# cvigilv/SimSpread.jl

Hardware: AMD Instinct MI355X
Metric: predicted edges/sec + achieved HBM GB/s, W*R SpMM (higher is better)
Workload: dtype f32

## Files before the change

### simspread.jl_amd/csrc/api.hip

```cpp
#include <algorithm>
#include <cmath>
#include <cstdlib>
#include <mutex>
#include <new>
#include <shared_mutex>
#include <type_traits>

#include "graph.hpp"

namespace ss {

std::string& last_error() {
  static thread_local std::string msg;
  return msg;
}

int fail(int code, const char* fmt, ...) {
  char buf[1024];
  va_list ap;
  va_start(ap, fmt);
  vsnprintf(buf, sizeof(buf), fmt, ap);
  va_end(ap);
  last_error() = buf;
  return code;
// ... 175 lines not shown
  T* dst = W;
  int64_t sld = ld, dld = ldw;
  if (mem == SS_MEM_HOST) {
    SS_TRY(din.alloc((size_t)rows * cols));
    SS_TRY(dout.alloc((size_t)rows * cols));
    SS_HIP(hipMemcpy2DAsync(din.p, rows * sizeof(T), G, ld * sizeof(T), rows * sizeof(T), cols, hipMemcpyHostToDevice, st));
    src = din.p; dst = dout.p; sld = rows; dld = rows;
  }
  SS_TRY(launch_row_degree<T>(src, rows, cols, sld, deg.p));
  SS_TRY(launch_spread_dense<T>(src, rows, cols, sld, deg.p, dst, dld));
  if (mem == SS_MEM_HOST)
    SS_HIP(hipMemcpy2DAsync(W, ldw * sizeof(T), dout.p, rows * sizeof(T), rows * sizeof(T), cols, hipMemcpyDeviceToHost, st));
  SS_HIP(hipStreamSynchronize(st));
  return SS_OK;
}

struct HandleHead {
  int dtype;
  std::mutex mu;
};
static uint64_t next_graph_id() {
  static std::atomic<uint64_t> n{0};
  return ++n;
}
template <class T>
struct GraphBox : HandleHead {
  uint64_t id = next_graph_id();
  Graph<T> g;
};
template <class T>
struct QueriesBox : HandleHead {
  uint64_t graph_id = 0;
  DevCsr<T> Xq;
};
template <class T>
struct SpMatBox : HandleHead {
  SpMat<T> m;
};

template <class T>
static int graph_check(const void* h, Graph<T>** out) {
  if (!h) return fail(SS_EINVAL, "graph handle is NULL");
  GraphBox<T>* b = const_cast<GraphBox<T>*>(reinterpret_cast<const GraphBox<T>*>(h));
  if (b->dtype != (int)sizeof(T)) return fail(SS_EINVAL, "graph handle was created with the other precision");
  *out = &b->g;
  return SS_OK;
}

template <class T>
static int queries_check(const void* qh, const void* h, const DevCsr<T>** out) {
  const QueriesBox<T>* q = reinterpret_cast<const QueriesBox<T>*>(qh);
  if (q->dtype != (int)sizeof(T)) return fail(SS_EINVAL, "query set was created with the other precision");
  if (q->graph_id != reinterpret_cast<const GraphBox<T>*>(h)->id)
    return fail(SS_EINVAL, "query set was created for another graph");
  *out = &q->Xq;
  return SS_OK;
}

template <class T>
static int graph_create_csr_impl(int64_t nq, int64_t ns, int64_t nf, int64_t nt, const int64_t* xq_ptr,
                                 const int32_t* xq_idx, const T* xq_val, const int64_t* xs_ptr, const int32_t* xs_idx,
                                 const T* xs_val, const int64_t* ys_ptr, const int32_t* ys_idx, const T* ys_val,
                                 int index_base, int mem, ss_graph** out) {
  SS_TRY(require_init());
  SS_TRY(check_mem(mem));
  if (!out) return fail(SS_EINVAL, "out handle pointer is NULL");
  *out = nullptr;
  if (nq < 0 || ns < 0 || nf < 0 || nt < 0) return fail(SS_EINVAL, "negative node count");
  GraphBox<T>* box = new (std::nothrow) GraphBox<T>();
  if (!box) return fail(SS_ENOMEM, "host allocation failed");
  box->dtype = (int)sizeof(T);
  Graph<T>& g = box->g;
  g.nq = nq; g.ns = ns; g.nf = nf; g.nt = nt;
  int rc = csr_from_user<T>(nq, nf, xq_ptr, xq_idx, xq_val, index_base, mem, g.Xq);
  if (rc == SS_OK) rc = csr_from_user<T>(ns, nf, xs_ptr, xs_idx, xs_val, index_base, mem, g.Xs);
  if (rc == SS_OK) rc = csr_from_user<T>(ns, nt, ys_ptr, ys_idx, ys_val, index_base, mem, g.Ys);
  if (rc == SS_OK) rc = graph_finalize<T>(g);
  if (rc != SS_OK) { delete box; return rc; }
  *out = reinterpret_cast<ss_graph*>(box);
  return SS_OK;
}

template <class T>
static int graph_create_dense_impl(int64_t nq, int64_t ns, int64_t nf, int64_t nt, const T* Sq, int64_t ldq,
                                   const T* Ss, int64_t lds, const T* Y, int64_t ldy, int apply_cutoff, T alpha,
                                   int weighted, int mem, ss_graph** out) {
  SS_TRY(require_init());
  SS_TRY(check_mem(mem));
// ... 812 lines not shown
    StageTimer t2(ST_SPMM);
    SS_TRY(launch_spmm_sell<T>(W, R, ldr, nb, out, d.ld, kt_clean, rows));
    timing_count(ST_NSPMM, 1);
    return SS_OK;
  }
  const size_t nsorted = (size_t)rb * (size_t)W.vrows;
  const size_t need_s = nsorted + (rows ? (size_t)rb * (size_t)ncols : 0);
  if (ws.n < need_s) SS_TRY(ws.alloc(need_s));
  {
    StageTimer t2(ST_SPMM);
    SS_TRY(launch_spmm_sell<T>(W, R, ldr, nb, ws.p, W.vrows, nullptr));
    timing_count(ST_NSPMM, 1);
  }
  StageTimer t3(ST_EPILOGUE);
  T* packed = ws.p + nsorted;
  SS_TRY(launch_unpermute<T>(ws.p, W.vrows, nb, ncols, W.vfirst.p, W.inv.p, kt_clean, rows ? packed : out,
                             rows ? ncols : d.ld));
  if (d.host_rows) {
    for (int64_t q = 0; q < nb; ++q)
      SS_HIP(hipMemcpyAsync(d.dst + (int64_t)d.host_rows[d.o + q] * d.ld, packed + q * ncols, ncols * sizeof(T),
                            hipMemcpyDeviceToDevice, ctx().stream));
  } else if (rows) {
    SS_TRY(launch_scatter_rows<T>(packed, ncols, nb, ncols, rows, d.dst, d.ld));
  }
  return SS_OK;
}

template <class T>
static int stage2_rows(Graph<T>& g, int64_t rb, int64_t nb, const int* kt_clean, const ScoreDest<T>& d) {
  return sell_rows<T>(g.W, g.Tws.p, g.ns, g.nt, g.Sws, rb, nb, kt_clean, d);
}

template <class T>
static int predict_rows_device(Graph<T>& g, const DevCsr<T>& Xq, int kind, int64_t row_begin, int64_t row_end, int clean,
                               T* dev_out, int64_t ldo) {
  const int64_t nrows = row_end - row_begin;
  const int64_t nj = g.ns;
  SS_TRY(graph_sell(g));
  SS_TRY(graph_chunked(g, kind == SS_ROWS_SOURCE));
  const int64_t rb = transfer_batch_rows(nrows, nj, sizeof(T));
  const size_t need = (size_t)rb * (size_t)(nj > 0 ? nj : 1);
  if (g.Tws.n < need) SS_TRY(g.Tws.alloc(need));
  DevBuf<T>& Tbuf = g.Tws;
  for (int64_t r0 = 0; r0 < nrows; r0 += rb) {
    const int64_t nb = (nrows - r0 < rb) ? (nrows - r0) : rb;
    {
      StageTimer t1(ST_TRANSFER);
      if (g.dense.on) {
        const bool loo = (kind == 2);
        const bool srcrows = (kind == SS_ROWS_SOURCE);
        SS_TRY(dense_transfer<T>(g, loo, loo ? g.dense.inv_kf_m1.p : g.inv_kf.p, g.inv_ks.p, g.ks.p, row_begin + r0, nb,
                                 Tbuf.p, nj, srcrows, nullptr));
        if (srcrows) {
          const DevCsr<T>* L[2] = {&g.Ys, nullptr};
          const DevChunked<T>* M[2] = {&g.YsTc, nullptr};
          const T* inv1[2] = {g.inv_kt.p, nullptr};
          SS_TRY(launch_transfer<T>(1, L, inv1, M, g.inv_ks.p, row_begin + r0, nb, nj, Tbuf.p, nj, nullptr, true));
        }
      } else if (kind == 2) {
        SS_TRY(launch_transfer_loo<T>(g.Xs, g.XsTc, g.kf.p, g.ks.p, row_begin + r0, nb, Tbuf.p, nj));
      } else if (kind == SS_ROWS_QUERY) {
        const bool want_block = env_int("SS_TRANSFER_V", 0) >= 2 && transfer_block_fits<T>(g.XsT.rows, g.XsTc.SC);
        if (want_block) {
          if (g.XsTb.SC == 0) {
            const int al = env_int("SS_TRANSFER_ALIGN", 32) == 1 ? 1 : 32;
            SS_TRY(chunked_build<T>(g.XsT, g.XsTc.SC, al, g.XsTb));
          }
          if (g.Cq.n < (size_t)(Xq.nnz > 0 ? Xq.nnz : 1)) SS_TRY(g.Cq.alloc((size_t)(Xq.nnz > 0 ? Xq.nnz : 1)));
          const bool fixed = !env_off("SS_TRANSFER_FIX");
          SS_TRY(launch_transfer_block<T>(Xq, g.inv_kf.p, g.XsTb, g.inv_ks.p, row_begin + r0, nb, nj, Tbuf.p, nj, g.Cq.p,
                                          g.XsTb.vmax, fixed));
        } else {
          const DevCsr<T>* L[2] = {&Xq, nullptr};
          const DevChunked<T>* M[2] = {&g.XsTc, nullptr};
          const T* inv1[2] = {g.inv_kf.p, nullptr};
          SS_TRY(launch_transfer<T>(1, L, inv1, M, g.inv_ks.p, row_begin + r0, nb, nj, Tbuf.p, nj));
        }
      } else {
        const DevCsr<T>* L[2] = {&g.Xs, &g.Ys};
        const DevChunked<T>* M[2] = {&g.XsTc, &g.YsTc};
        const T* inv1[2] = {g.inv_kf.p, g.inv_kt.p};
        SS_TRY(launch_transfer<T>(2, L, inv1, M, g.inv_ks.p, row_begin + r0, nb, nj, Tbuf.p, nj));
      }
      timing_count(ST_NTRANSFER, 1);
    }
    SS_TRY(stage2_rows<T>(g, rb, nb, clean ? g.kt.p : nullptr, ScoreDest<T>{dev_out, ldo, r0, nullptr, nullptr}));
  }
  if (kind == 2 && clean) {
    StageTimer t3(ST_EPILOGUE);
    SS_TRY(launch_loo_clean_fix<T>(g.YsT, g.kt.p, row_begin, nrows, dev_out, ldo));
  }
  return SS_OK;
}

template <class T>
static int loo_graph_check(const Graph<T>& g) {
  if (g.general || (!g.dense.on && g.nq != 0) || g.ns != g.nf)
    return fail(SS_EINVAL, "leave-one-out needs a graph with nq == 0 and ns == nf (feature j named after source j)");
  return SS_OK;
}

template <class T>
struct ScoreOut {
  T* out = nullptr;
  int64_t ld = 0, nrows = 0, nt = 0;
  int layout = SS_LAYOUT_ROWMAJOR, mem = SS_MEM_DEVICE;
  T* dev_rm = nullptr;
  int64_t ld_rm = 0;
  hipEvent_t e_begin = nullptr;
  DevBuf<T> scores;
  DevBuf<T> cm;

  bool direct() const { return mem == SS_MEM_DEVICE && layout == SS_LAYOUT_ROWMAJOR; }
  int begin(T* out_, int64_t ld_, int layout_, int mem_, int64_t nrows_, int64_t nt_) {
    out = out_; ld = ld_; layout = layout_; mem = mem_; nrows = nrows_; nt = nt_;
// ... 17 lines not shown
        SS_TRY(cm.alloc((size_t)nrows * nt));
        dst = cm.p;
        dld = nrows;
      }
      SS_TRY(launch_transpose<T>(dev_rm, nrows, nt, ld_rm, dst, dld));
    }
    hipEvent_t e_end;
    SS_TRY(timing_mark(&e_end));
    timing_span(ST_TOTAL, e_begin, e_end);
    if (mem == SS_MEM_HOST) {
      StageTimer t5(ST_D2H);
      if (layout == SS_LAYOUT_ROWMAJOR) {
        SS_HIP(hipMemcpy2DAsync(out, ld * sizeof(T), dev_rm, ld_rm * sizeof(T), nt * sizeof(T), nrows,
                                hipMemcpyDeviceToHost, ctx().stream));
      } else {
        SS_HIP(hipMemcpy2DAsync(out, ld * sizeof(T), cm.p, nrows * sizeof(T), nrows * sizeof(T), nt,
                                hipMemcpyDeviceToHost, ctx().stream));
      }
    }
    return SS_OK;
  }
};

template <class T>
static int predict_impl(ss_graph* h, int kind, int64_t row_begin, int64_t row_end, int clean, T* out, int64_t ld,
                        int layout, int mem, const ss_queries* qh = nullptr) {
  SS_TRY(require_init());
  SS_TRY(check_mem(mem));
  SS_TRY(check_layout(layout));
  Graph<T>* gp = nullptr;
  SS_TRY(graph_check<T>(h, &gp));
  Graph<T>& g = *gp;
  const DevCsr<T>* xq = &g.Xq;
  if (qh) SS_TRY(queries_check<T>(qh, h, &xq));
  const int64_t limit = (kind == SS_ROWS_QUERY) ? (qh ? xq->rows : g.nq) : g.ns;
  if (g.general && kind != SS_ROWS_QUERY)
    return fail(SS_EINVAL, "a general graph serves SS_ROWS_QUERY only");
  if (kind == 2) {
    SS_TRY(loo_graph_check(g));
  } else if (kind != SS_ROWS_QUERY && kind != SS_ROWS_SOURCE) {
    return fail(SS_EINVAL, "rows_kind must be SS_ROWS_QUERY or SS_ROWS_SOURCE");
  }
  if (row_begin < 0 || row_end < row_begin || row_end > limit)
    return fail(SS_EINVAL, "row range [%lld,%lld) outside 0..%lld", (long long)row_begin, (long long)row_end,
                (long long)limit);
  const int64_t nrows = row_end - row_begin;
  const int64_t nt = g.nt;
  if (nrows == 0 || nt == 0) return SS_OK;
  if (!out) return fail(SS_EINVAL, "output buffer is NULL");
  const int64_t need_ld = (layout == SS_LAYOUT_ROWMAJOR) ? nt : nrows;
  if (ld < need_ld) return fail(SS_EINVAL, "leading dimension %lld < %lld", (long long)ld, (long long)need_ld);
  ScoreOut<T> so;
  SS_TRY(so.begin(out, ld, layout, mem, nrows, nt));
  SS_TRY(predict_rows_device<T>(g, *xq, kind, row_begin, row_end, clean, so.dev_rm, so.ld_rm));
  SS_TRY(so.deliver());
  if (!so.direct()) SS_HIP(hipStreamSynchronize(ctx().stream));
  return SS_OK;
}

static int check_rank_rows_shape(int64_t ncols, int L, double alpha) {
  if (ncols < 2 || ncols >= (1LL << 31) - 1)
    return fail(SS_EINVAL, "rank metrics rows: ncols = %lld outside [2, 2^31 - 1)", (long long)ncols);
  if (L < 1) return fail(SS_EINVAL, "Please use a list length greater than 0 (L > 0)");
  if ((int64_t)L >= ncols) return fail(SS_EINVAL, "Number of labels is less than length (L > y)");
  if (!(alpha > 0.0)) return fail(SS_EINVAL, "rank metrics rows: alpha must be positive");
  return SS_OK;
}

template <class T>
struct StagedRows {
  std::vector<int64_t> hp;
  const int64_t* dptr = nullptr;
  const int* didx = nullptr;
  const T* dyhat = nullptr;
  int64_t shift = 0, dld = 0, nnz = 0;
  DevBuf<int64_t> bptr;
  DevBuf<int> bidx;
  DevBuf<T> bhat;
};

template <class T>
static int stage_label_rows(const char* what, const int64_t* yptr, const int32_t* yidx, int base, const T* yhat,
                            int64_t nrows, int64_t ncols, int64_t ld, int mem, StagedRows<T>& s) {
  hipStream_t st = ctx().stream;
  std::vector<int64_t>& hp = s.hp;
  hp.resize((size_t)nrows + 1);
  if (mem == SS_MEM_HOST) memcpy(hp.data(), yptr, hp.size() * sizeof(int64_t));
// ... 3503 lines not shown
```

### simspread.jl_amd/csrc/assemble.hip

```cpp
#include <cstdlib>
#include <cstring>
#include <hip/hip_runtime.h>
#include <rocprim/rocprim.hpp>

#include "graph.hpp"

namespace ss {

static inline int grid_for(int64_t work, int block, int cap = 256 * 16) {
  int64_t g = ceil_div(work, block);
  if (g < 1) g = 1;
  if (g > cap) g = cap;
  return (int)g;
}

__global__ void scan_tail_kernel(const int* in, int* out, int64_t n) { out[n] = out[n - 1] + in[n - 1]; }

static int exclusive_scan_int(const int* in, int* out, int64_t n) {
  hipStream_t st = ctx().stream;
  if (n == 0) {
    SS_HIP(hipMemsetAsync(out, 0, sizeof(int), st));
    return SS_OK;
  }
  size_t bytes = 0;
// ... 1215 lines not shown
  SS_TRY(out.idx.alloc(out.stored + 256));
  SS_TRY(out.val.alloc(out.stored + 256));
  SS_HIP(hipMemsetAsync(out.idx.p + out.stored, 0, 256 * sizeof(unsigned short), st));
  SS_HIP(hipMemsetAsync(out.val.p + out.stored, 0, 256 * sizeof(T), st));
  const int sched = ((align == 1 || align == 32) && !env_off("SS_CHUNK_SCHED")) ? 1 : 0;
  hipLaunchKernelGGL(chunk_fill_kernel<T>, dim3(grid_for(total * 64, 256)), dim3(256), 0, st, in.ptr.p, in.idx.p,
                     in.val.p, in.rows, SC, out.nchunks, align, sched, out.off.p, out.idx.p, out.val.p);
  SS_LAUNCH_CHECK();
  SS_HIP(hipStreamSynchronize(st));
  return SS_OK;
}

template <class T>
__global__ void degree_kernel(const int* __restrict__ pa, const int* __restrict__ pb, int64_t n, int* __restrict__ k,
                              T* __restrict__ inv) {
  for (int64_t i = (int64_t)blockIdx.x * blockDim.x + threadIdx.x; i < n; i += (int64_t)gridDim.x * blockDim.x) {
    int d = pa[i + 1] - pa[i];
    if (pb) d += pb[i + 1] - pb[i];
    k[i] = d;
    inv[i] = d > 0 ? T(1) / T(d) : T(0);
  }
}

template <class T>
int graph_finalize(Graph<T>& g) {
  SS_TRY(csr_transpose(g.Xs, g.XsT));
  SS_TRY(csr_transpose(g.Ys, g.YsT));
  return graph_degrees(g);
}

template <class T>
int graph_degrees(Graph<T>& g) {
  hipStream_t st = ctx().stream;
  SS_TRY(g.kf.alloc(g.nf));
  SS_TRY(g.ks.alloc(g.ns));
  SS_TRY(g.kt.alloc(g.nt));
  SS_TRY(g.inv_kf.alloc(g.nf));
  SS_TRY(g.inv_ks.alloc(g.ns));
  SS_TRY(g.inv_kt.alloc(g.nt));
  if (g.nf > 0) {
    hipLaunchKernelGGL(degree_kernel<T>, dim3(grid_for(g.nf, 256)), dim3(256), 0, st, g.XsT.ptr.p, (const int*)nullptr,
                       g.nf, g.kf.p, g.inv_kf.p);
    SS_LAUNCH_CHECK();
  }
  if (g.ns > 0) {
    hipLaunchKernelGGL(degree_kernel<T>, dim3(grid_for(g.ns, 256)), dim3(256), 0, st, g.Xs.ptr.p, g.Ys.ptr.p, g.ns,
                       g.ks.p, g.inv_ks.p);
    SS_LAUNCH_CHECK();
  }
  if (g.nt > 0) {
    hipLaunchKernelGGL(degree_kernel<T>, dim3(grid_for(g.nt, 256)), dim3(256), 0, st, g.YsT.ptr.p, (const int*)nullptr,
                       g.nt, g.kt.p, g.inv_kt.p);
    SS_LAUNCH_CHECK();
  }
  SS_HIP(hipStreamSynchronize(st));
  return SS_OK;
}

template <class T>
int graph_finalize_general(Graph<T>& g) {
  hipStream_t st = ctx().stream;
  const int64_t n = g.ns;
  SS_TRY(g.kf.alloc(n));
  SS_TRY(g.inv_kf.alloc(n));
  SS_TRY(g.ks.alloc(n));
  SS_TRY(g.inv_ks.alloc(n));
  SS_TRY(g.kt.alloc(g.nt));
  SS_TRY(g.inv_kt.alloc(g.nt));
  if (n > 0) {
    hipLaunchKernelGGL(degree_kernel<T>, dim3(grid_for(n, 256)), dim3(256), 0, st, g.XsT.ptr.p, (const int*)nullptr, n,
                       g.kf.p, g.inv_kf.p);
    SS_LAUNCH_CHECK();
    hipLaunchKernelGGL(degree_kernel<T>, dim3(grid_for(n, 256)), dim3(256), 0, st, g.XsT.ptr.p, (const int*)nullptr, n,
                       g.ks.p, g.inv_ks.p);
    SS_LAUNCH_CHECK();
  }
  if (g.nt > 0) {
    hipLaunchKernelGGL(degree_kernel<T>, dim3(grid_for(g.nt, 256)), dim3(256), 0, st, g.YsT.ptr.p, (const int*)nullptr,
                       g.nt, g.kt.p, g.inv_kt.p);
    SS_LAUNCH_CHECK();
  }
  SS_HIP(hipStreamSynchronize(st));
  return SS_OK;
}

template <class T>
int graph_finalize_general_targets(Graph<T>& g) {
  hipStream_t st = ctx().stream;
  SS_TRY(g.kt.alloc(g.nt));
  SS_TRY(g.inv_kt.alloc(g.nt));
  if (g.nt > 0) {
    hipLaunchKernelGGL(degree_kernel<T>, dim3(grid_for(g.nt, 256)), dim3(256), 0, st, g.YsT.ptr.p,
                       (const int*)nullptr, g.nt, g.kt.p, g.inv_kt.p);
    SS_LAUNCH_CHECK();
  }
  SS_HIP(hipStreamSynchronize(st));
  return SS_OK;
}

#define SS_INSTANTIATE(T)                                                                                      \
  template int graph_finalize_general_targets<T>(Graph<T>&);                                                    \
  template int csr_from_user<T>(int64_t, int64_t, const int64_t*, const int32_t*, const T*, int, int, DevCsr<T>&); \
  template int csr_from_dense<T>(const T*, int64_t, int64_t, int64_t, bool, T, bool, int, DevCsr<T>&);         \
  template int csr_transpose<T>(const DevCsr<T>&, DevCsr<T>&);                                                 \
  template int chunked_build<T>(const DevCsr<T>&, int, int, DevChunked<T>&);                                     \
  template int sell_build<T>(const DevCsr<T>&, int, DevSell<T>&, int);                                            \
  template int graph_finalize<T>(Graph<T>&);                                                                   \
  template int graph_degrees<T>(Graph<T>&);                                                                    \
  template int graph_finalize_general<T>(Graph<T>&);
SS_INSTANTIATE(float)
SS_INSTANTIATE(double)

}
```

### simspread.jl_amd/csrc/dense.hip

```cpp
#include "graph.hpp"

namespace ss {

template <class T>
__device__ __forceinline__ T cut_val(T x, T alpha, int weighted) {
  return (x >= alpha) ? (weighted ? x : T(1)) : T(0);
}

template <class T>
__global__ void dense_col_degree_kernel(const T* __restrict__ S, int64_t rows, int64_t cols, int64_t ld,
                                        T alpha, int weighted, int* __restrict__ deg) {
  const int lane = threadIdx.x & 63;
  const int64_t wave0 = ((int64_t)blockIdx.x * blockDim.x + threadIdx.x) >> 6;
  const int64_t nwaves = ((int64_t)gridDim.x * blockDim.x) >> 6;
  for (int64_t f = wave0; f < cols; f += nwaves) {
    int n = 0;
    for (int64_t r = lane; r < rows; r += 64) n += cut_val(S[r + f * ld], alpha, weighted) != T(0) ? 1 : 0;
    for (int o = 32; o > 0; o >>= 1) n += __shfl_xor(n, o);
    if (lane == 0) deg[f] = n;
  }
}

template <class T>
__global__ void dense_row_degree_kernel(const T* __restrict__ S, int64_t rows, int64_t cols, int64_t ld,
// ... 246 lines not shown
  const int lane = threadIdx.x & 63;
  const int64_t wave0 = ((int64_t)blockIdx.x * blockDim.x + threadIdx.x) >> 6;
  const int64_t nwaves = ((int64_t)gridDim.x * blockDim.x) >> 6;
  for (int64_t m = wave0; m < nm; m += nwaves) {
    const int g = members[m];
    for (int x = yptr[g] + lane; x < yptr[g + 1]; x += 64) atomicSub(&kt[yidx[x]], 1);
  }
}

template <class T>
int dense_fold_degrees(const Graph<T>& g, const int* members, int64_t nm, int* kf, int* ks, int* kt) {
  if (nm <= 0) return SS_OK;
  const DenseSim<T>& d = g.dense;
  hipStream_t st = ctx().stream;
  const auto cap = [](int64_t x) { return (unsigned)(x < 1 ? 1 : (x > 4096 ? 4096 : x)); };
  hipLaunchKernelGGL(dense_fold_kf_kernel<T>, dim3(cap(ceil_div(d.nf * 64, 256))), dim3(256), 0, st, d.Ss.p, d.ns, d.nf,
                     d.alpha, d.weighted ? 1 : 0, members, nm, kf);
  SS_LAUNCH_CHECK();
  hipLaunchKernelGGL(dense_fold_ks_kernel<T>, dim3(cap(ceil_div(d.ns, 256))), dim3(256), 0, st, d.Ss.p, d.ns, d.ns, d.alpha,
                     d.weighted ? 1 : 0, members, nm, ks);
  SS_LAUNCH_CHECK();
  hipLaunchKernelGGL(dense_fold_kt_kernel, dim3(cap(ceil_div(nm * 64, 256))), dim3(256), 0, st, g.Ys.ptr.p, g.Ys.idx.p,
                     members, nm, kt);
  SS_LAUNCH_CHECK();
  return SS_OK;
}

template <class T>
int dense_degrees(Graph<T>& g) {
  hipStream_t st = ctx().stream;
  DenseSim<T>& d = g.dense;
  DevBuf<int> kx;
  SS_TRY(kx.alloc(d.ns));
  SS_TRY(g.kf.alloc(d.nf));
  SS_TRY(g.inv_kf.alloc(d.nf));
  SS_TRY(d.inv_kf_m1.alloc(d.nf));
  SS_TRY(g.ks.alloc(d.ns));
  SS_TRY(g.inv_ks.alloc(d.ns));
  if (d.ns > 0 && d.nf > 0) {
    DevBuf<int> kcol;
    SS_TRY(kcol.alloc(d.nf));
    hipLaunchKernelGGL(dense_col_degree_kernel<T>, dim3((unsigned)(ceil_div(d.nf * 64, 256) < 4096 ? ceil_div(d.nf * 64, 256) : 4096)),
                       dim3(256), 0, st, d.Ss.p, d.ns, d.nf, d.ns, d.alpha, d.weighted ? 1 : 0, kcol.p);
    SS_LAUNCH_CHECK();
    SS_HIP(hipMemsetAsync(kx.p, 0, d.ns * sizeof(int), st));
    int nsplit = (int)ceil_div(65536, d.ns);
    if (nsplit < 1) nsplit = 1;
    if (nsplit > d.nf) nsplit = (int)d.nf;
    if (nsplit > 1024) nsplit = 1024;
    const int64_t cps = ceil_div(d.nf, nsplit);
    nsplit = (int)ceil_div(d.nf, cps);
    hipLaunchKernelGGL(dense_row_degree_kernel<T>, dim3((unsigned)ceil_div(d.ns, 64), (unsigned)nsplit), dim3(64), 0, st,
                       d.Ss.p, d.ns, d.nf, d.ns, d.alpha, d.weighted ? 1 : 0, cps, kx.p);
    SS_LAUNCH_CHECK();
    hipLaunchKernelGGL(dense_finish_degrees_kernel<T>, dim3((unsigned)ceil_div(d.nf, 256)), dim3(256), 0, st, kcol.p,
                       (const int*)nullptr, d.nf, g.kf.p, g.inv_kf.p, d.inv_kf_m1.p);
    SS_LAUNCH_CHECK();
    hipLaunchKernelGGL(dense_finish_degrees_kernel<T>, dim3((unsigned)ceil_div(d.ns, 256)), dim3(256), 0, st, kx.p,
                       g.Ys.ptr.p, d.ns, g.ks.p, g.inv_ks.p, (T*)nullptr);
    SS_LAUNCH_CHECK();
  }
  SS_HIP(hipStreamSynchronize(st));
  return SS_OK;
}

template int dense_degrees<float>(Graph<float>&);
// ... 6 lines not shown
```

### simspread.jl_amd/csrc/graph.hpp

```cpp
#pragma once
#include "common.hpp"

#include <type_traits>

namespace ss {

template <class T>
struct DevCsr {
  int64_t rows = 0, cols = 0, nnz = 0;
  DevBuf<int> ptr;
  DevBuf<int> idx;
  DevBuf<T> val;
  bool binary = false;
};

constexpr int SELL_Q1_STEP = 8;
constexpr int SELL_LEND_R = 3;
constexpr unsigned SELL_REC_NONE = 0x00ffffffu;

template <class T>
struct DevSell {
  int64_t rows = 0, cols = 0;
  int KC = 0;
  int qt = 0;
// ... 27 lines not shown
  DevBuf<unsigned short> len;
  bool len_ok = false;
  float vmax = 0.f, vmin = 0.f;
};

template <class T>
struct DevCsell {
  int64_t rows = 0, cols = 0, nnz = 0;
  int KC = 0, nchunks = 0, nslices = 0;
  int QT = 0;
  bool binary = false;
  bool ok = false;
  int64_t npairs = 0;
  DevBuf<int> desc;
  DevBuf<unsigned short> np;
  DevBuf<unsigned> pidx;
  DevBuf<T> pval;
};

template <class T>
struct DenseSim {
  bool on = false;
  int64_t nq = 0, ns = 0, nf = 0;
  T alpha = T(0);
  bool weighted = true;
  DevBuf<T> Sq, Ss;
  DevBuf<T> inv_kf_m1;
  DevBuf<unsigned short> Bpl, Apl;
  int Bpl_np = 0;
  int64_t Bpl_Np = 0, Bpl_Kp = 0;
};

template <class T>
struct Graph {
  int64_t nq = 0, ns = 0, nf = 0, nt = 0;
  bool general = false;
  DenseSim<T> dense;
  DevCsr<T> Xq;
  DevCsr<T> Xs;
  DevCsr<T> XsT;
  DevCsr<T> Ys;
  DevCsr<T> YsT;
  DevBuf<int> kf, ks, kt;
  DevBuf<T> inv_kf, inv_ks, inv_kt;
  DevSell<T> W;
  int W_qt = 0;
  DevChunked<T> XsTc, YsTc;
  DevChunked<T> XsTb;
  DevBuf<T> Cq;
  DevBuf<T> Tws;
  DevBuf<T> Sws;
};

template <class T>
struct SpMat {
  DevCsr<T> csr;
  DevSell<T> sell;
  int sell_qt = 0;
  DevChunked<T> narrow[3];
  DevChunked<T> col[3];
  DevCsell<T> csell[6];
  bool csell_tried[6] = {false, false, false, false, false, false};
  DevBuf<T> partial;
};

template <class T>
int csr_from_user(int64_t rows, int64_t cols, const int64_t* ptr, const int32_t* idx, const T* val,
                  int index_base, int mem, DevCsr<T>& out);
template <class T>
int csr_from_dense(const T* S, int64_t rows, int64_t cols, int64_t ld, bool apply_cutoff, T alpha,
                   bool weighted, int mem, DevCsr<T>& out);
template <class T>
int csr_transpose(const DevCsr<T>& in, DevCsr<T>& out);
template <class T>
int sell_build(const DevCsr<T>& in, int KCmax, DevSell<T>& out, int qt = 0);
template <class T>
int chunked_build(const DevCsr<T>& in, int SC, int align, DevChunked<T>& out);
template <class T>
int csell_build(const DevCsr<T>& in, int KC, int QT, DevCsell<T>& out);
template <class T>
int graph_finalize(Graph<T>& g);
template <class T>
int graph_degrees(Graph<T>& g);
template <class T>
int graph_finalize_general(Graph<T>& g);
template <class T>
int graph_finalize_general_targets(Graph<T>& g);

template <class T>
struct CsrView {
  const int* ptr;
  const int* idx;
  const T* val;
};
template <class T>
inline CsrView<T> view(const DevCsr<T>& m) { return CsrView<T>{m.ptr.p, m.idx.p, m.val.p}; }

template <class T>
int launch_cutoff(const T* X, int64_t rows, int64_t cols, int64_t ld, T alpha, bool weighted, T* out, int64_t ldo);
template <class T>
int launch_row_degree(const T* G, int64_t rows, int64_t cols, int64_t ld, int* deg);
template <class T>
int launch_spread_dense(const T* G, int64_t rows, int64_t cols, int64_t ld, const int* deg, T* W, int64_t ldw);

template <class T>
int launch_transfer(int nterms, const DevCsr<T>* L[2], const T* inv1[2], const DevChunked<T>* Mt[2],
                    const T* inv2, int64_t row_begin, int64_t nrows, int64_t nj, T* out, int64_t ld,
                    const int* row_ids = nullptr, bool accumulate = false);
template <class T>
int launch_transfer_block(const DevCsr<T>& L, const T* inv1, const DevChunked<T>& Mt, const T* inv2, int64_t row_begin,
                          int64_t nrows, int64_t nj, T* out, int64_t ld, T* coef, float xmax, bool fixed);
template <class T>
bool transfer_block_fits(int64_t mrows, int SC);
template <class T>
int launch_fold_degrees(const DevCsr<T>& X, const DevCsr<T>& XT, const DevCsr<T>& Y, const int* members,
                        int64_t nmembers, int* kf, int* ks, int* kt);
template <class T>
int launch_fold_inverse(const int* kf, const int* ks, const int* fold, int phi, int64_t nf, int64_t ns, T* inv_kf,
                        T* inv_ks);
template <class T>
int launch_transfer_loo(const DevCsr<T>& X, const DevChunked<T>& XT, const int* kf, const int* ks,
                        int64_t i_begin, int64_t nrows, T* out, int64_t ld);

template <class T>
int sell_tile_width();
template <class T>
int sell_max_chunk(int qt);
template <class T>
int launch_spmm_sell(const DevSell<T>& W, const T* R, int64_t ldr, int64_t B, T* F, int64_t ldf,
                     const int* clean_deg, const int* out_rows = nullptr);
template <class T>
int narrow_chunk_cols(int bv);
template <class T>
int launch_spmm_chunked_narrow(const DevChunked<T>& W, int bv, const T* R, int64_t ldr, int B, T* F, int64_t ldf,
                               DevBuf<T>& partial);
int csell_chunk_cols(int rowb);
template <class T>
int launch_spmm_csell(const DevCsell<T>& W, const T* R, int64_t ldr, int B, T* F, int64_t ldf, DevBuf<T>& partial);
template <class T>
int colgroup_chunk_cols(int bv);
template <class T>
int launch_spmm_colgroup(const DevChunked<T>& W, int bv, const T* R, int64_t ldr, int B, T* F, int64_t ldf,
                         DevBuf<T>& partial);

template <class T>
int launch_jaccard(const T* F, int64_t n, int64_t d, int64_t ld, T* S, int64_t lds);

int launch_topl(const float* scores, int64_t nrows, int64_t ncols, int64_t ld, int L, int* oidx, float* oval);
int launch_rank_metrics(const unsigned char* y, const float* yhat, int64_t n, double alpha, double* out4);

template <class PtrT>
int launch_rank_rows_validate(const PtrT* yptr, int64_t shift, const int* yidx, int base, int64_t nrows, int64_t ncols);
template <class T, class PtrT>
int launch_rank_rows(const PtrT* yptr, int64_t shift, const int* yidx, int base, const PtrT* host_ptr, const T* yhat,
                     int64_t nrows, int64_t ncols, int64_t ld, double alpha, int L, double* out);
// ... 264 lines not shown
```

### simspread.jl_amd/csrc/transfer.hip

```cpp
#include <type_traits>

#include "graph.hpp"

namespace ss {

template <class T>
struct ChunkedView {
  const int* off;
  const unsigned short* idx;
  const T* val;
  int64_t rows;
};
template <class T>
static inline ChunkedView<T> view(const DevChunked<T>& m) {
  return ChunkedView<T>{m.off.p, m.idx.p, m.val.p, m.rows};
}

template <class T>
struct TransferArgs {
  int nterms;
  CsrView<T> L[2];
  const T* inv1[2];
  ChunkedView<T> M[2];
  const T* inv2;
  const int* kf;
  const int* ks;
  int64_t row_begin;
  const int* row_ids;
  int64_t nj;
  int SC;
  int nchunks;
  T* out;
  int64_t ld;
  int accumulate;
  float xmax;
  int chunk_interleave;
};
template <class T>
__device__ __forceinline__ bool chunks_in_turn(const TransferArgs<T>& p) { return p.chunk_interleave != 0; }

template <class F>
static int dispatch_bool(bool b, F&& f) {
  return b ? f(std::true_type{}) : f(std::false_type{});
}
template <int... Vs, class F>
static int dispatch_int(int v, F&& f) {
  int rc = SS_OK;
  const bool hit = ((v == Vs && ((rc = f(std::integral_constant<int, Vs>{})), true)) || ...);
  return hit ? rc : fail(SS_EINVAL, "dispatch_int: no kernel for the value %d", v);
}

template <auto Kernel, class... Args>
static int launch_lds(unsigned grid, int block, size_t lds, Args... args) {
  static std::atomic<bool> attr_done{false};
  if (!attr_done) {
// ... 185 lines not shown
  }
  unsigned long long m = __ballot(n_l > 80);
  while (m != 0ull) {
    const int src = __builtin_ctzll(m);
    m &= m - 1ull;
    const int n = __builtin_amdgcn_readlane(n_l, src);
    const unsigned b = (unsigned)__builtin_amdgcn_readlane(b_l, src);
    const T cf = BitsOf<T>::bcast(cf_l, src);
    for (int x = 80 + lane; x < n; x += 64) {
      const int j = midx[b + x];
      const T v = BINM ? T(1) : mval[b + x];
      if constexpr (FIX) atomicAdd(reinterpret_cast<unsigned*>(acc) + j, (unsigned)cvt_rpi((float)(cf * v)));
      else acc[j] = fma(cf, v, acc[j]);
    }
  }
}

struct FixedScale {
  float scale, unscale;
};
template <class F>
__device__ __forceinline__ FixedScale fixed_scale(int lb, int le, int lane, float xmax, F&& abs_coef) {
  float sabs = 0.f;
  for (int q = lb + lane; q < le; q += 64) sabs += abs_coef(q);
#pragma unroll
  for (int o = 32; o > 0; o >>= 1) sabs += __shfl_xor(sabs, o);
  int e = 0;
  (void)frexpf(sabs * xmax, &e);
  if (!(sabs * xmax > 0.f)) e = 0;
  e = e < -90 ? -90 : (e > 120 ? 120 : e);
  return FixedScale{ldexpf(1.f, 30 - e), ldexpf(1.f, e - 30)};
}

template <class T, bool LOO, int U, bool BINM, bool DUAL, bool FIX = false, bool BUF = false>
__global__ void __launch_bounds__(TRANSFER_THREADS) transfer_kernel(TransferArgs<T> p) {
  static_assert(64 % (2 * U) == 0, "U must divide 32");
  extern __shared__ __align__(16) unsigned char smem_raw[];
  T* acc = reinterpret_cast<T*>(smem_raw);
  const int astride = p.SC + 64;
  constexpr int NCOPY = DUAL ? 2 : 1;
  unsigned* bits = reinterpret_cast<unsigned*>(acc + NCOPY * astride);
  const int lane = threadIdx.x;
  int c;
  int64_t r;
  if (p.nchunks > 8 && p.nchunks % 8 == 0 && !chunks_in_turn(p)) {
    const int64_t nrows = (int64_t)gridDim.x / p.nchunks, per = nrows * 8;
    const int64_t grp = blockIdx.x / per, rem = blockIdx.x - grp * per;
    r = rem >> 3;
    c = (int)(grp * 8 + (rem & 7));
  } else {
    c = blockIdx.x % p.nchunks;
    r = blockIdx.x / p.nchunks;
  }
  const int64_t gr = p.row_ids ? (int64_t)p.row_ids[p.row_begin + r] : p.row_begin + r;
  const int64_t j0 = (int64_t)c * p.SC;
  const int jn = (int)((p.nj - j0 < p.SC) ? (p.nj - j0) : p.SC);
  const int dummy = p.SC + lane;

  for (int j = lane; j < NCOPY * astride; j += 64) acc[j] = T(0);
  if (LOO)
    for (int j = lane; j < (p.SC + 31) / 32; j += 64) bits[j] = 0u;
  __syncthreads();

  float fix_unscale = 1.f;
  for (int t = 0; t < p.nterms; ++t) {
    const CsrView<T> L = p.L[t];
    const ChunkedView<T> M = p.M[t];
    const int* __restrict__ off = M.off + (int64_t)c * M.rows;
    const unsigned short* __restrict__ midx = M.idx;
    const T* __restrict__ mval = M.val;
    const int lb = L.ptr[gr], le = L.ptr[gr + 1];
    float scale = 1.f;
    if constexpr (FIX) {
      float sabs = 0.f;
      for (int q = lb + lane; q < le; q += 64) sabs += fabsf((float)(L.val[q] * p.inv1[t][L.idx[q]]));
#pragma unroll
      for (int o = 32; o > 0; o >>= 1) sabs += __shfl_xor(sabs, o);
      int e = 0;
      (void)frexpf(sabs * p.xmax, &e);
      if (!(sabs * p.xmax > 0.f)) e = 0;
      e = e < -90 ? -90 : (e > 120 ? 120 : e);
      scale = ldexpf(1.f, 30 - e);
      fix_unscale = ldexpf(1.f, e - 30);
    }
    for (int g0 = lb; g0 < le; g0 += 64) {
      const int q = g0 + lane;
      int b_l = 0, n_l = 0;
      T cf_l = T(0);
      if (q < le) {
        const int a = L.idx[q];
        const T lv = L.val[q];
        if (LOO) {
          const int d = p.kf[a] - 1;
          cf_l = (a != (int)gr && d > 0) ? lv * (T(1) / T(d)) : T(0);
        } else {
          cf_l = lv * p.inv1[t][a];
          if constexpr (FIX) cf_l = (T)((float)cf_l * scale);
        }
        if (cf_l != T(0)) { b_l = off[a]; n_l = off[a + 1] - b_l; }
      }
      const int cnt = __builtin_amdgcn_readfirstlane((le - g0 < 64) ? (le - g0) : 64);
      SubRows<T, U> A, B;
      auto load = [&](SubRows<T, U>& sr, int first) __attribute__((always_inline)) {
        if constexpr (BUF) {
          const __amdgpu_buffer_rsrc_t ridx = __builtin_amdgcn_make_buffer_rsrc((void*)midx, 0, -1, 0x00020000);
          const __amdgpu_buffer_rsrc_t rval = __builtin_amdgcn_make_buffer_rsrc((void*)mval, 0, -1, 0x00020000);
          subrows_load_buf<U, BINM>(sr, first, b_l, n_l, cf_l, ridx, rval, lane);
        } else {
          subrows_load<T, U, BINM>(sr, first, b_l, n_l, cf_l, midx, mval, lane);
        }
      };
      auto tail_ld = [&](unsigned e, unsigned short& j, T& v) __attribute__((always_inline)) {
        if constexpr (BUF) {
          const __amdgpu_buffer_rsrc_t ridx = __builtin_amdgcn_make_buffer_rsrc((void*)midx, 0, -1, 0x00020000);
          const __amdgpu_buffer_rsrc_t rval = __builtin_amdgcn_make_buffer_rsrc((void*)mval, 0, -1, 0x00020000);
          j = __builtin_amdgcn_raw_buffer_load_b16(ridx, (int)(e * 2u), 0, 0);
          v = BINM ? 1.f : __builtin_bit_cast(float, __builtin_amdgcn_raw_buffer_load_b32(rval, (int)(e * 4u), 0, 0));
        } else {
          j = midx[e];
          v = BINM ? T(1) : mval[e];
        }
      };
// ... 647 lines not shown
            return launch_block_kernel<TB_WIDE2, transfer_wide2_kernel<decltype(B)::value>>(p, Mt, coef, nrows, n, xmax);
          });
        }
      } else if (wide > 0) {
        if (const int n = transfer_block_waves<TB_WIDE, T>(Mt.rows, Mt.SC)) {
          path_add("wide");
          return dispatch_int<2, 4>(wide == 2 ? 2 : 4, [&](auto D) {
            return dispatch_bool(binm, [&](auto B) {
              return launch_block_kernel<TB_WIDE, transfer_wide_kernel<decltype(D)::value, decltype(B)::value>>(
                  p, Mt, coef, nrows, n, xmax);
            });
          });
        }
      } else if (const int n = transfer_block_waves<TB_QFLAT, T>(Mt.rows, Mt.SC)) {
        path_add("qflat");
        return dispatch_bool(binm, [&](auto B) {
          return launch_block_kernel<TB_QFLAT, transfer_qflat_kernel<float, 4, decltype(B)::value>>(p, Mt, coef, nrows, n, xmax);
        });
      }
    }
  }
  return dispatch_int<4, 8>(transfer_u() == 4 ? 4 : 8, [&](auto U) {
    return dispatch_bool(binm, [&](auto B) {
      return dispatch_bool(fx, [&](auto F) {
        constexpr bool FIX = CANFIX && decltype(F)::value;
        return launch_block_kernel<TB_PLAIN, transfer_block_kernel<T, decltype(U)::value, decltype(B)::value, FIX>>(
            p, Mt, coef, nrows, nw, xmax);
      });
    });
  });
}

template <class T, bool LOO>
static int launch_transfer_variant(const TransferArgs<T>& p, unsigned grid, size_t lds, bool binm, bool dual) {
  auto launch = [&](auto kernel) {
    hipLaunchKernelGGL(kernel, dim3(grid), dim3(TRANSFER_THREADS), lds, ctx().stream, p);
    SS_LAUNCH_CHECK();
    return (int)SS_OK;
  };
  const int u = transfer_u();
  if constexpr (std::is_same<T, float>::value && !LOO) {
    const bool buf = !dual && env_int("SS_TRANSFER_LD", 0) == 1;
    const bool fix = !dual && env_int("SS_TRANSFER_FIX1", 0) == 1 && p.nterms == 1 && !p.accumulate;
    if (buf) path_add("buffer_loads");
    if (fix) path_add("fixed_point");
    if (buf || fix)
      return dispatch_int<4, 8>(u == 4 ? 4 : 8, [&](auto U) {
        return dispatch_bool(binm, [&](auto B) {
          return dispatch_bool(fix, [&](auto F) {
            return dispatch_bool(buf, [&](auto BF) {
              return launch(transfer_kernel<T, LOO, decltype(U)::value, decltype(B)::value, false, decltype(F)::value,
                                            decltype(BF)::value>);
            });
          });
        });
      });
  }
  return dispatch_int<4, 8, 16>(u, [&](auto U) {
    return dispatch_bool(binm, [&](auto B) {
      return dispatch_bool(dual, [&](auto D) {
        return launch(transfer_kernel<T, LOO, decltype(U)::value, decltype(B)::value, decltype(D)::value>);
      });
    });
  });
}

template <class T>
int launch_transfer(int nterms, const DevCsr<T>* L[2], const T* inv1[2], const DevChunked<T>* Mt[2],
                    const T* inv2, int64_t row_begin, int64_t nrows, int64_t nj, T* out, int64_t ld,
                    const int* row_ids, bool accumulate) {
  if (nrows <= 0 || nj <= 0) return SS_OK;
  TransferArgs<T> p{};
  p.nterms = nterms;
  for (int t = 0; t < nterms; ++t) {
    p.L[t] = view(*L[t]);
    p.M[t] = view(*Mt[t]);
    p.inv1[t] = inv1[t];
    if (Mt[t]->SC != Mt[0]->SC || Mt[t]->nchunks != Mt[0]->nchunks)
      return fail(SS_EINVAL, "transfer operands were cut with different chunk sizes");
  }
  p.inv2 = inv2;
  p.row_begin = row_begin;
  p.row_ids = row_ids;
  p.nj = nj;
  p.SC = Mt[0]->SC;
  p.nchunks = Mt[0]->nchunks;
  p.out = out;
  p.ld = ld;
  p.accumulate = accumulate ? 1 : 0;
  p.xmax = 1.0f;
  p.chunk_interleave = env_off("SS_TRANSFER_ORDER") ? 1 : 0;
  bool binm = true;
  for (int t = 0; t < nterms; ++t) binm = binm && Mt[t]->binary;
  const int64_t grid = nrows * p.nchunks;
  if (grid >= (1LL << 31)) return fail(SS_EUNSUPPORTED, "transfer grid too large; lower SS_TRANSFER_BYTES");
  const bool dual = transfer_dual();
  path_add("transfer");
  const size_t lds = (size_t)(p.SC + 64) * sizeof(T) * (dual ? 2 : 1);
  return launch_transfer_variant<T, false>(p, (unsigned)grid, lds, binm, dual);
}

template <class T>
int launch_transfer_loo(const DevCsr<T>& X, const DevChunked<T>& XT, const int* kf, const int* ks,
                        int64_t i_begin, int64_t nrows, T* out, int64_t ld) {
  if (nrows <= 0) return SS_OK;
  TransferArgs<T> p{};
  p.nterms = 1;
  p.L[0] = view(X);
  p.M[0] = view(XT);
  p.kf = kf;
  p.ks = ks;
  p.row_begin = i_begin;
  p.nj = X.rows;
  p.SC = XT.SC;
  p.nchunks = XT.nchunks;
  p.out = out;
  p.ld = ld;
  p.chunk_interleave = env_off("SS_TRANSFER_ORDER") ? 1 : 0;
  const int64_t grid = nrows * p.nchunks;
  if (grid >= (1LL << 31)) return fail(SS_EUNSUPPORTED, "transfer grid too large; lower SS_TRANSFER_BYTES");
  const bool dual = transfer_dual();
  path_add("transfer_loo");
  const size_t lds = (size_t)(p.SC + 64) * sizeof(T) * (dual ? 2 : 1) + (size_t)((p.SC + 31) / 32) * 4;
  return launch_transfer_variant<T, true>(p, (unsigned)grid, lds, XT.binary, dual);
}

#define SS_INSTANTIATE(T)                                                                                   \
  template int launch_transfer<T>(int, const DevCsr<T>*[2], const T*[2], const DevChunked<T>*[2], const T*, \
                                  int64_t, int64_t, int64_t, T*, int64_t, const int*, bool);                      \
  template int launch_transfer_block<T>(const DevCsr<T>&, const T*, const DevChunked<T>&, const T*, int64_t, int64_t, \
                                        int64_t, T*, int64_t, T*, float, bool);                               \
  template bool transfer_block_fits<T>(int64_t, int);                                                        \
  template int launch_transfer_loo<T>(const DevCsr<T>&, const DevChunked<T>&, const int*, const int*,       \
                                      int64_t, int64_t, T*, int64_t);
SS_INSTANTIATE(float)
SS_INSTANTIATE(double)

}
```

Baseline: 51.66 billion.

## Cache per-nonzero transfer coefficients in a device table reused across predict calls

Precomputes, for each nonzero of the left CSR operand, the product of its value and the inverse degree (or the leave-one-out coefficient) into a device table kept on the graph or query handle. It is invalidated by an epoch bump whenever degrees change. The transfer kernel gets a COEF variant that reads the precomputed coefficient instead of gathering inv1/kf per nonzero, which removes a dependent indirect load and a division from the inner setup. This costs extra device memory equal to the operand's nnz and an initial build kernel, and the table persists across calls.

New measurement: 52.66 billion (median of 6 runs). 1.9% higher.

```diff
diff --git a/simspread.jl_amd/csrc/api.hip b/simspread.jl_amd/csrc/api.hip
--- a/simspread.jl_amd/csrc/api.hip
+++ b/simspread.jl_amd/csrc/api.hip
@@ -231,6 +231,7 @@
 struct QueriesBox : HandleHead {
   uint64_t graph_id = 0;
   DevCsr<T> Xq;
+  CoefTable<T> coef;
 };
 template <class T>
 struct SpMatBox : HandleHead {
@@ -247,12 +248,13 @@
 }
 
 template <class T>
-static int queries_check(const void* qh, const void* h, const DevCsr<T>** out) {
-  const QueriesBox<T>* q = reinterpret_cast<const QueriesBox<T>*>(qh);
+static int queries_check(const void* qh, const void* h, const DevCsr<T>** out, CoefTable<T>** tab = nullptr) {
+  QueriesBox<T>* q = const_cast<QueriesBox<T>*>(reinterpret_cast<const QueriesBox<T>*>(qh));
   if (q->dtype != (int)sizeof(T)) return fail(SS_EINVAL, "query set was created with the other precision");
   if (q->graph_id != reinterpret_cast<const GraphBox<T>*>(h)->id)
     return fail(SS_EINVAL, "query set was created for another graph");
   *out = &q->Xq;
+  if (tab) *tab = &q->coef;
   return SS_OK;
 }
 
@@ -1131,12 +1133,41 @@
 }
 
 template <class T>
+static int coef_table(const Graph<T>& g, CoefTable<T>& tb, const DevCsr<T>& L, const T* inv1, const int* kf_loo,
+                      const T** out) {
+  *out = nullptr;
+  if (env_off("SS_TRANSFER_COEF")) return SS_OK;
+  const int64_t cap = env_int("SS_TRANSFER_COEF_BYTES", 1LL << 30);
+  if (L.nnz * (int64_t)sizeof(T) > cap) return SS_OK;
+  if (tb.epoch != g.coef_epoch) {
+    tb.drop();
+    SS_TRY(tb.c.alloc((size_t)L.nnz));
+    SS_TRY(transfer_coef_build<T>(L, inv1, kf_loo, tb.c.p));
+    tb.epoch = g.coef_epoch;
+  }
+  *out = tb.c.p;
+  return SS_OK;
+}
+
+template <class T>
 static int predict_rows_device(Graph<T>& g, const DevCsr<T>& Xq, int kind, int64_t row_begin, int64_t row_end, int clean,
-                               T* dev_out, int64_t ldo) {
+                               T* dev_out, int64_t ldo, CoefTable<T>* qtab = nullptr) {
   const int64_t nrows = row_end - row_begin;
   const int64_t nj = g.ns;
   SS_TRY(graph_sell(g));
   SS_TRY(graph_chunked(g, kind == SS_ROWS_SOURCE));
+  const T* coef[2] = {nullptr, nullptr};
+  if (!g.dense.on) {
+    if (kind == 2) {
+      SS_TRY(coef_table<T>(g, g.coef_loo, g.Xs, nullptr, g.kf.p, &coef[0]));
+    } else if (kind == SS_ROWS_QUERY) {
+      if (&Xq == &g.Xq) qtab = &g.coef_q;
+      if (qtab) SS_TRY(coef_table<T>(g, *qtab, Xq, g.inv_kf.p, nullptr, &coef[0]));
+    } else {
+      SS_TRY(coef_table<T>(g, g.coef_s, g.Xs, g.inv_kf.p, nullptr, &coef[0]));
+      SS_TRY(coef_table<T>(g, g.coef_y, g.Ys, g.inv_kt.p, nullptr, &coef[1]));
+    }
+  }
   const int64_t rb = transfer_batch_rows(nrows, nj, sizeof(T));
   const size_t need = (size_t)rb * (size_t)(nj > 0 ? nj : 1);
   if (g.Tws.n < need) SS_TRY(g.Tws.alloc(need));
@@ -1157,7 +1188,7 @@
           SS_TRY(launch_transfer<T>(1, L, inv1, M, g.inv_ks.p, row_begin + r0, nb, nj, Tbuf.p, nj, nullptr, true));
         }
       } else if (kind == 2) {
-        SS_TRY(launch_transfer_loo<T>(g.Xs, g.XsTc, g.kf.p, g.ks.p, row_begin + r0, nb, Tbuf.p, nj));
+        SS_TRY(launch_transfer_loo<T>(g.Xs, g.XsTc, g.kf.p, g.ks.p, row_begin + r0, nb, Tbuf.p, nj, coef[0]));
       } else if (kind == SS_ROWS_QUERY) {
         const bool want_block = env_int("SS_TRANSFER_V", 0) >= 2 && transfer_block_fits<T>(g.XsT.rows, g.XsTc.SC);
         if (want_block) {
@@ -1173,13 +1204,13 @@
           const DevCsr<T>* L[2] = {&Xq, nullptr};
           const DevChunked<T>* M[2] = {&g.XsTc, nullptr};
           const T* inv1[2] = {g.inv_kf.p, nullptr};
-          SS_TRY(launch_transfer<T>(1, L, inv1, M, g.inv_ks.p, row_begin + r0, nb, nj, Tbuf.p, nj));
+          SS_TRY(launch_transfer<T>(1, L, inv1, M, g.inv_ks.p, row_begin + r0, nb, nj, Tbuf.p, nj, nullptr, false, coef));
         }
       } else {
         const DevCsr<T>* L[2] = {&g.Xs, &g.Ys};
         const DevChunked<T>* M[2] = {&g.XsTc, &g.YsTc};
         const T* inv1[2] = {g.inv_kf.p, g.inv_kt.p};
-        SS_TRY(launch_transfer<T>(2, L, inv1, M, g.inv_ks.p, row_begin + r0, nb, nj, Tbuf.p, nj));
+        SS_TRY(launch_transfer<T>(2, L, inv1, M, g.inv_ks.p, row_begin + r0, nb, nj, Tbuf.p, nj, nullptr, false, coef));
       }
       timing_count(ST_NTRANSFER, 1);
     }
@@ -1263,7 +1294,8 @@
   SS_TRY(graph_check<T>(h, &gp));
   Graph<T>& g = *gp;
   const DevCsr<T>* xq = &g.Xq;
-  if (qh) SS_TRY(queries_check<T>(qh, h, &xq));
+  CoefTable<T>* qtab = nullptr;
+  if (qh) SS_TRY(queries_check<T>(qh, h, &xq, &qtab));
   const int64_t limit = (kind == SS_ROWS_QUERY) ? (qh ? xq->rows : g.nq) : g.ns;
   if (g.general && kind != SS_ROWS_QUERY)
     return fail(SS_EINVAL, "a general graph serves SS_ROWS_QUERY only");
@@ -1283,7 +1315,7 @@
   if (ld < need_ld) return fail(SS_EINVAL, "leading dimension %lld < %lld", (long long)ld, (long long)need_ld);
   ScoreOut<T> so;
   SS_TRY(so.begin(out, ld, layout, mem, nrows, nt));
-  SS_TRY(predict_rows_device<T>(g, *xq, kind, row_begin, row_end, clean, so.dev_rm, so.ld_rm));
+  SS_TRY(predict_rows_device<T>(g, *xq, kind, row_begin, row_end, clean, so.dev_rm, so.ld_rm, qtab));
   SS_TRY(so.deliver());
   if (!so.direct()) SS_HIP(hipStreamSynchronize(ctx().stream));
   return SS_OK;
diff --git a/simspread.jl_amd/csrc/assemble.hip b/simspread.jl_amd/csrc/assemble.hip
--- a/simspread.jl_amd/csrc/assemble.hip
+++ b/simspread.jl_amd/csrc/assemble.hip
@@ -1271,6 +1271,7 @@
 template <class T>
 int graph_degrees(Graph<T>& g) {
   hipStream_t st = ctx().stream;
+  g.coef_drop();
   SS_TRY(g.kf.alloc(g.nf));
   SS_TRY(g.ks.alloc(g.ns));
   SS_TRY(g.kt.alloc(g.nt));
@@ -1300,6 +1301,7 @@
 int graph_finalize_general(Graph<T>& g) {
   hipStream_t st = ctx().stream;
   const int64_t n = g.ns;
+  g.coef_drop();
   SS_TRY(g.kf.alloc(n));
   SS_TRY(g.inv_kf.alloc(n));
   SS_TRY(g.ks.alloc(n));
@@ -1326,6 +1328,7 @@
 template <class T>
 int graph_finalize_general_targets(Graph<T>& g) {
   hipStream_t st = ctx().stream;
+  g.coef_drop();
   SS_TRY(g.kt.alloc(g.nt));
   SS_TRY(g.inv_kt.alloc(g.nt));
   if (g.nt > 0) {
diff --git a/simspread.jl_amd/csrc/dense.hip b/simspread.jl_amd/csrc/dense.hip
--- a/simspread.jl_amd/csrc/dense.hip
+++ b/simspread.jl_amd/csrc/dense.hip
@@ -302,6 +302,7 @@
   DenseSim<T>& d = g.dense;
   DevBuf<int> kx;
   SS_TRY(kx.alloc(d.ns));
+  g.coef_drop();
   SS_TRY(g.kf.alloc(d.nf));
   SS_TRY(g.inv_kf.alloc(d.nf));
   SS_TRY(d.inv_kf_m1.alloc(d.nf));
diff --git a/simspread.jl_amd/csrc/graph.hpp b/simspread.jl_amd/csrc/graph.hpp
--- a/simspread.jl_amd/csrc/graph.hpp
+++ b/simspread.jl_amd/csrc/graph.hpp
@@ -83,6 +83,13 @@
 };
 
 template <class T>
+struct CoefTable {
+  DevBuf<T> c;
+  uint64_t epoch = 0;
+  void drop() { c.release(); epoch = 0; }
+};
+
+template <class T>
 struct Graph {
   int64_t nq = 0, ns = 0, nf = 0, nt = 0;
   bool general = false;
@@ -99,6 +106,12 @@
   DevChunked<T> XsTc, YsTc;
   DevChunked<T> XsTb;
   DevBuf<T> Cq;
+  CoefTable<T> coef_q, coef_s, coef_y, coef_loo;
+  uint64_t coef_epoch = 1;
+  void coef_drop() {
+    coef_q.drop(); coef_s.drop(); coef_y.drop(); coef_loo.drop();
+    ++coef_epoch;
+  }
   DevBuf<T> Tws;
   DevBuf<T> Sws;
 };
@@ -157,7 +170,9 @@
 template <class T>
 int launch_transfer(int nterms, const DevCsr<T>* L[2], const T* inv1[2], const DevChunked<T>* Mt[2],
                     const T* inv2, int64_t row_begin, int64_t nrows, int64_t nj, T* out, int64_t ld,
-                    const int* row_ids = nullptr, bool accumulate = false);
+                    const int* row_ids = nullptr, bool accumulate = false, const T* const* coef = nullptr);
+template <class T>
+int transfer_coef_build(const DevCsr<T>& L, const T* inv1, const int* kf_loo, T* coef);
 template <class T>
 int launch_transfer_block(const DevCsr<T>& L, const T* inv1, const DevChunked<T>& Mt, const T* inv2, int64_t row_begin,
                           int64_t nrows, int64_t nj, T* out, int64_t ld, T* coef, float xmax, bool fixed);
@@ -171,7 +186,7 @@
                         T* inv_ks);
 template <class T>
 int launch_transfer_loo(const DevCsr<T>& X, const DevChunked<T>& XT, const int* kf, const int* ks,
-                        int64_t i_begin, int64_t nrows, T* out, int64_t ld);
+                        int64_t i_begin, int64_t nrows, T* out, int64_t ld, const T* coef = nullptr);
 
 template <class T>
 int sell_tile_width();
diff --git a/simspread.jl_amd/csrc/transfer.hip b/simspread.jl_amd/csrc/transfer.hip
--- a/simspread.jl_amd/csrc/transfer.hip
+++ b/simspread.jl_amd/csrc/transfer.hip
@@ -21,6 +21,7 @@
   int nterms;
   CsrView<T> L[2];
   const T* inv1[2];
+  const T* coef[2];
   ChunkedView<T> M[2];
   const T* inv2;
   const int* kf;
@@ -272,9 +273,10 @@
   return FixedScale{ldexpf(1.f, 30 - e), ldexpf(1.f, e - 30)};
 }
 
-template <class T, bool LOO, int U, bool BINM, bool DUAL, bool FIX = false, bool BUF = false>
+template <class T, bool LOO, int U, bool BINM, bool DUAL, bool FIX = false, bool BUF = false, bool COEF = false>
 __global__ void __launch_bounds__(TRANSFER_THREADS) transfer_kernel(TransferArgs<T> p) {
   static_assert(64 % (2 * U) == 0, "U must divide 32");
+  static_assert(!COEF || (!DUAL && !FIX && !BUF), "coefficient tables serve the default family only");
   extern __shared__ __align__(16) unsigned char smem_raw[];
   T* acc = reinterpret_cast<T*>(smem_raw);
   const int astride = p.SC + 64;
@@ -327,7 +329,15 @@
       const int q = g0 + lane;
       int b_l = 0, n_l = 0;
       T cf_l = T(0);
-      if (q < le) {
+      if constexpr (COEF) {
+        if (q < le) {
+          const int a = L.idx[q];
+          cf_l = p.coef[t][q];
+          const int o0 = off[a], o1 = off[a + 1];
+          b_l = o0;
+          n_l = cf_l != T(0) ? o1 - o0 : 0;
+        }
+      } else if (q < le) {
         const int a = L.idx[q];
         const T lv = L.val[q];
         if (LOO) {
@@ -1041,6 +1051,44 @@
 }
 
 template <class T, bool LOO>
+__global__ void __launch_bounds__(256) transfer_coef_rows_kernel(CsrView<T> L, const T* __restrict__ inv1,
+                                                                 const int* __restrict__ kf, int64_t nrows,
+                                                                 T* __restrict__ coef) {
+  for (int64_t r = blockIdx.x; r < nrows; r += gridDim.x) {
+    const int lb = L.ptr[r], le = L.ptr[r + 1];
+    for (int q = lb + (int)threadIdx.x; q < le; q += 256) {
+      const int a = L.idx[q];
+      const T lv = L.val[q];
+      if (LOO) {
+        const int d = kf[a] - 1;
+        coef[q] = (a != (int)r && d > 0) ? lv * (T(1) / T(d)) : T(0);
+      } else {
+        coef[q] = lv * inv1[a];
+      }
+    }
+  }
+}
+
+template <class T>
+int transfer_coef_build(const DevCsr<T>& L, const T* inv1, const int* kf_loo, T* coef) {
+  if (L.rows <= 0 || L.nnz <= 0) return SS_OK;
+  const unsigned grid = (unsigned)(L.rows < 65536 ? L.rows : 65536);
+  if (kf_loo)
+    hipLaunchKernelGGL((transfer_coef_rows_kernel<T, true>), dim3(grid), dim3(256), 0, ctx().stream, view(L), inv1, kf_loo,
+                       L.rows, coef);
+  else
+    hipLaunchKernelGGL((transfer_coef_rows_kernel<T, false>), dim3(grid), dim3(256), 0, ctx().stream, view(L), inv1, kf_loo,
+                       L.rows, coef);
+  SS_LAUNCH_CHECK();
+  return SS_OK;
+}
+
+static int transfer_coef_mode() {
+  const int m = (int)env_int("SS_TRANSFER_COEF", 1);
+  return m == 0 ? 0 : (m == 2 ? 2 : 1);
+}
+
+template <class T, bool LOO>
 static int launch_transfer_variant(const TransferArgs<T>& p, unsigned grid, size_t lds, bool binm, bool dual) {
   auto launch = [&](auto kernel) {
     hipLaunchKernelGGL(kernel, dim3(grid), dim3(TRANSFER_THREADS), lds, ctx().stream, p);
@@ -1048,6 +1096,18 @@
     return (int)SS_OK;
   };
   const int u = transfer_u();
+  bool coef = !dual && (u == 4 || u == 8) && transfer_coef_mode() != 0 && p.row_ids == nullptr;
+  if constexpr (std::is_same<T, float>::value && !LOO)
+    coef = coef && env_int("SS_TRANSFER_LD", 0) != 1 && env_int("SS_TRANSFER_FIX1", 0) != 1;
+  for (int t = 0; t < p.nterms; ++t) coef = coef && p.coef[t] != nullptr;
+  if (coef) {
+    if (transfer_coef_mode() == 2) path_add("coef_table");
+    return dispatch_int<4, 8>(u, [&](auto U) {
+      return dispatch_bool(binm, [&](auto B) {
+        return launch(transfer_kernel<T, LOO, decltype(U)::value, decltype(B)::value, false, false, false, true>);
+      });
+    });
+  }
   if constexpr (std::is_same<T, float>::value && !LOO) {
     const bool buf = !dual && env_int("SS_TRANSFER_LD", 0) == 1;
     const bool fix = !dual && env_int("SS_TRANSFER_FIX1", 0) == 1 && p.nterms == 1 && !p.accumulate;
@@ -1077,7 +1137,7 @@
 template <class T>
 int launch_transfer(int nterms, const DevCsr<T>* L[2], const T* inv1[2], const DevChunked<T>* Mt[2],
                     const T* inv2, int64_t row_begin, int64_t nrows, int64_t nj, T* out, int64_t ld,
-                    const int* row_ids, bool accumulate) {
+                    const int* row_ids, bool accumulate, const T* const* coef) {
   if (nrows <= 0 || nj <= 0) return SS_OK;
   TransferArgs<T> p{};
   p.nterms = nterms;
@@ -1085,6 +1145,7 @@
     p.L[t] = view(*L[t]);
     p.M[t] = view(*Mt[t]);
     p.inv1[t] = inv1[t];
+    p.coef[t] = coef ? coef[t] : nullptr;
     if (Mt[t]->SC != Mt[0]->SC || Mt[t]->nchunks != Mt[0]->nchunks)
       return fail(SS_EINVAL, "transfer operands were cut with different chunk sizes");
   }
@@ -1111,7 +1172,7 @@
 
 template <class T>
 int launch_transfer_loo(const DevCsr<T>& X, const DevChunked<T>& XT, const int* kf, const int* ks,
-                        int64_t i_begin, int64_t nrows, T* out, int64_t ld) {
+                        int64_t i_begin, int64_t nrows, T* out, int64_t ld, const T* coef) {
   if (nrows <= 0) return SS_OK;
   TransferArgs<T> p{};
   p.nterms = 1;
@@ -1119,6 +1180,7 @@
   p.M[0] = view(XT);
   p.kf = kf;
   p.ks = ks;
+  p.coef[0] = coef;
   p.row_begin = i_begin;
   p.nj = X.rows;
   p.SC = XT.SC;
@@ -1136,12 +1198,13 @@
 
 #define SS_INSTANTIATE(T)                                                                                   \
   template int launch_transfer<T>(int, const DevCsr<T>*[2], const T*[2], const DevChunked<T>*[2], const T*, \
-                                  int64_t, int64_t, int64_t, T*, int64_t, const int*, bool);                      \
+                                  int64_t, int64_t, int64_t, T*, int64_t, const int*, bool, const T* const*);     \
+  template int transfer_coef_build<T>(const DevCsr<T>&, const T*, const int*, T*);                          \
   template int launch_transfer_block<T>(const DevCsr<T>&, const T*, const DevChunked<T>&, const T*, int64_t, int64_t, \
                                         int64_t, T*, int64_t, T*, float, bool);                               \
   template bool transfer_block_fits<T>(int64_t, int);                                                        \
   template int launch_transfer_loo<T>(const DevCsr<T>&, const DevChunked<T>&, const int*, const int*,       \
-                                      int64_t, int64_t, T*, int64_t);
+                                      int64_t, int64_t, T*, int64_t, const T*);
 SS_INSTANTIATE(float)
 SS_INSTANTIATE(double)
 
```
